# THU-luvision/TextureFusion

Measured on AMD Instinct MI355X. Metric: RGB-D frames/s (TSDF integrate + atlas update: prepare->integrate->finalize, UpdateMeshes, GeneratePatches + UpdateAtlas over the frame's dirty chunks), higher is better.
Workload: dtype f32

## Files before the change

texturefusion_amd/csrc/tf_devfn.h:

```cpp
#pragma once

#include "tf_device.h"

namespace tf {

__device__ __forceinline__ unsigned long long pack_id(int x, int y, int z) {
  return ((unsigned long long)((uint32_t)(x + (1 << 20)) & 0x1FFFFFu) << 42) |
         ((unsigned long long)((uint32_t)(y + (1 << 20)) & 0x1FFFFFu) << 21) |
         (unsigned long long)((uint32_t)(z + (1 << 20)) & 0x1FFFFFu);
}
__device__ __forceinline__ int4 unpack_id(unsigned long long k) {
  int4 r;
  r.x = (int)((k >> 42) & 0x1FFFFFu) - (1 << 20);
  r.y = (int)((k >> 21) & 0x1FFFFFu) - (1 << 20);
  r.z = (int)(k & 0x1FFFFFu) - (1 << 20);
  r.w = 0;
  return r;
}
__device__ __forceinline__ int part_key(const VolumeDev& v, int x, int y, int z) {
  return v.part_a * x + v.part_b * y + v.part_c * z;
}
__device__ __forceinline__ bool part_owned(const VolumeDev& v, int x, int y, int z) {
  const int k = part_key(v, x, y, z);
  return k >= v.part_lo && k < v.part_hi;
}
__device__ __forceinline__ bool part_band(const VolumeDev& v, int x, int y, int z) {
  const long long k = part_key(v, x, y, z);
  const long long s = v.part_a + v.part_b + v.part_c;
  return (k >= (long long)v.part_lo && k - (long long)v.part_lo <= s) || k == (long long)v.part_hi - 1;
}

__device__ __forceinline__ bool part_interior(const VolumeDev& v, int x, int y, int z) {
  const long long k = part_key(v, x, y, z);
  const long long s = (long long)v.part_a + v.part_b + v.part_c;
  return k - s >= (long long)v.part_lo && k + s < (long long)v.part_hi;
}

__device__ __forceinline__ uint32_t hash_key(unsigned long long k) {
  const unsigned long long h = k * 0x9E3779B97F4A7C15ull;
  return (uint32_t)(h >> 32) ^ (uint32_t)h;
}


__device__ __forceinline__ uint32_t hash_find(const VolumeDev& v, unsigned long long key) {
  uint32_t i = hash_key(key) & v.hmask;
  for (uint32_t probe = 0; probe <= v.hmask; ++probe) {
    const unsigned long long cur = v.hent[i].key;
    if (cur == key) return i;
    if (cur == kEmptyKey) return kInvalidSlot;
    i = (i + 1) & v.hmask;
  }
  return kInvalidSlot;
}

__device__ __forceinline__ uint32_t hash_slot_alive(const VolumeDev& v, unsigned long long key) {
  uint32_t i = hash_key(key) & v.hmask;
  for (uint32_t probe = 0; probe <= v.hmask; ++probe) {
    const uint4 e = *reinterpret_cast<const uint4*>(&v.hent[i]);
    const unsigned long long cur = ((unsigned long long)e.y << 32) | e.x;
    if (cur == key) return (e.w & 1u) ? e.z : kInvalidSlot;
    if (cur == kEmptyKey) return kInvalidSlot;
    i = (i + 1) & v.hmask;
  }
  return kInvalidSlot;
}

__device__ __forceinline__ uint32_t hash_slot_alive_ent(const VolumeDev& v, unsigned long long key, uint32_t* ent) {
  uint32_t i = hash_key(key) & v.hmask;
  for (uint32_t probe = 0; probe <= v.hmask; ++probe) {
    const uint4 e = *reinterpret_cast<const uint4*>(&v.hent[i]);
    const unsigned long long cur = ((unsigned long long)e.y << 32) | e.x;
    if (cur == key) { *ent = i; return (e.w & 1u) ? e.z : kInvalidSlot; }
    if (cur == kEmptyKey) return kInvalidSlot;
    i = (i + 1) & v.hmask;
  }
  return kInvalidSlot;
}

__device__ __forceinline__ uint32_t chunk_acquire(const VolumeDev& v, int4 id, bool* is_new,
                                               uint32_t* ent, const bool lazy = false) {
  const unsigned long long key = pack_id(id.x, id.y, id.z);
  uint32_t i = hash_key(key) & v.hmask;
  *is_new = true;
  for (uint32_t probe = 0; probe <= v.hmask; ++probe) {
    unsigned long long cur = v.hent[i].key;
    if (cur == kEmptyKey) {
      cur = atomicCAS(&v.hent[i].key, kEmptyKey, key);
      if (cur == kEmptyKey) {
        *ent = i;
        v.vctl->create_seq = v.seq;
        const uint32_t stripe = (hash_key(key) >> 7) & (kSlotStripes - 1);
        const uint32_t per = v.max_chunks / kSlotStripes;
        const uint32_t k = atomicAdd(&v.vctl->slot_cnt[stripe], 1u);
        const uint32_t slot = stripe * per + k;
        if (k >= per) {
          atomicOr(&v.vctl->status, kStPoolFull);
          v.hent[i].slot = kInvalidSlot;
          v.hent[i].alive = 0;
          return kInvalidSlot;
        }
        v.hent[i].slot = slot;
        v.hent[i].alive = 1;
        return slot;
      }
    }
    if (cur == key) {
      *ent = i;
      const uint32_t slot = v.hent[i].slot;
      if (slot == kInvalidSlot) return slot;
      if (!v.hent[i].alive) { if (!lazy) v.hent[i].alive = 1; }
      else *is_new = false;
      return slot;
    }
    i = (i + 1) & v.hmask;
  }
  atomicOr(&v.vctl->status, kStHashFull);
  *ent = 0;
  return kInvalidSlot;
}

__device__ __forceinline__ int nbr_word(int dx, int dy, int dz) { return (dx + 1) + 3 * (dy + 1) + 9 * (dz + 1); }
__device__ __forceinline__ uint32_t nbr_probe(const VolumeDev& v, unsigned long long key) {
  uint32_t i = hash_key(key) & v.hmask;
  for (uint32_t probe = 0; probe <= v.hmask; ++probe) {
    const uint4 e = *reinterpret_cast<const uint4*>(&v.hent[i]);
    const unsigned long long cur = ((unsigned long long)e.y << 32) | e.x;
    if (cur == key) return e.z + 1u;
    if (cur == kEmptyKey) return 0u;
    i = (i + 1) & v.hmask;
  }
  return 0u;
}
__device__ __forceinline__ uint32_t nbr_row_checked(const VolumeDev& v, const uint32_t own, const int4 id, const int lane,
                                                   uint32_t w, const uint32_t create_seq) {
  const uint32_t st = (uint32_t)__shfl((int)w, kNbrStamp);
  if (!(st > create_seq)) {
    if (lane < 27 && lane != 13 && w == 0u) {
      w = nbr_probe(v, pack_id(id.x + lane % 3 - 1, id.y + (lane / 3) % 3 - 1, id.z + lane / 9 - 1));
      if (w) v.nbr[(size_t)own * kNbrWords + lane] = w;
    }
    if (lane == kNbrStamp) v.nbr[(size_t)own * kNbrWords + lane] = v.seq;
  }
  return w;
}

constexpr uint32_t kBlkFail = 0x7FFFFFFFu;
__device__ __forceinline__ uint32_t blk_ring_mask(const VolumeDev& v, const int large) {
  uint32_t ns = v.mesh_blocks, nl = v.ovf_blocks;
  asm volatile("" : "+s"(ns), "+s"(nl));
  const uint32_t ms = ns > 2u ? (0xFFFFFFFFu >> __builtin_clz(ns - 1u)) : 1u;
  const uint32_t ml = nl > 2u ? (0xFFFFFFFFu >> __builtin_clz(nl - 1u)) : 1u;
  return large ? ml : ms;
}
__device__ __forceinline__ uint32_t* blk_ring(const VolumeDev& v, const int large) {
  uint32_t* const r = reinterpret_cast<uint32_t*>(v.mesh_rec + v.max_chunks);
// ... 88 lines not shown
```

texturefusion_amd/csrc/tf_kernels.hip:

```cpp
#include <stdlib.h>

#include <atomic>
#include "tf_device.h"
#include "tf_devfn.h"
#include "tf_devpose.h"
#include "tf_host_math.h"
#include "tf_patch_body.h"
#include "tf_voxel_math.h"

#pragma clang fp contract(off)
#ifndef TF_KA_GP
#define TF_KA_GP 2
#endif


namespace tf {

__global__ void k_reset_ctl(FrameCtl* ctl, VolCtl* vctl) {
  if (blockIdx.x == 0 && threadIdx.x == 0) {
    for (int a = 0; a < 3; ++a) {
      ctl->bbox_key[a] = f2key(1e8f);
      ctl->bbox_key[3 + a] = f2key(-1e8f);
      ctl->min_id[a] = ctl->max_id[a] = ctl->dims[a] = 0;
    }
// ... 432 lines not shown
    if (tile == n_tiles - 1u && threadIdx.x == 0) finish(tile_base + agg);
    __syncthreads();
  }
}
void launch_scan(const VolumeDev& v, int step, hipStream_t s) {
  static std::atomic<uint32_t> g_stamp{0};
  uint32_t stamp;
  do { stamp = (g_stamp.fetch_add(1u) + 1u) & 0x3FFFFFFFu; } while (stamp == 0u);
  hipLaunchKernelGGL(k_scan, dim3(256), dim3(256), 0, s, v, step, stamp);
}

__global__ __launch_bounds__(256) void k_acquire(VolumeDev v) {
  const SelBuf& L = v.sel;
  const uint32_t n = L.ctl->n_list;
  for (uint32_t e = blockIdx.x * 256 + threadIdx.x; e < n; e += gridDim.x * 256) {
    const int4 id = L.list_id[e];
    bool is_new = false;
    uint32_t ent = 0;
    const uint32_t slot = chunk_acquire(v, id, &is_new, &ent);
    L.list_slot[e] = slot;
    L.list_ent[e] = ent;
    L.list_new[e] = is_new ? 1 : 0;
    L.list_needs[e] = 0;
  }
}
void launch_acquire(const VolumeDev& v, hipStream_t s) {
  hipLaunchKernelGGL(k_acquire, dim3(512), dim3(256), 0, s, v);
}

__global__ __launch_bounds__(256) void k_pre(VolumeDev v, Pose P, Integ ig, float res, float resDiag, float4* out_pre,
                                             float* out_cen) {
  const SelBuf& L = v.sel;
  float4* pre = out_pre ? out_pre : L.list_pre;
  if (blockIdx.x == 0) centroid_table(P.p, res, out_cen ? out_cen : L.cen);
  const uint32_t n = L.ctl->n_list <= v.max_list ? L.ctl->n_list : 0u;
  for (uint32_t e = blockIdx.x * 256 + threadIdx.x; e < n; e += gridDim.x * 256) {
    const int4 id = L.list_id[e];
    const ChunkPre cp = chunk_pre(id, P.p, ig, res, resDiag);
    pre[4 * e] = make_float4(cp.a.x, cp.a.y, cp.a.z, cp.b.x);
    pre[4 * e + 1] = make_float4(cp.b.y, __int_as_float(id.x), __int_as_float(id.y), __int_as_float(id.z));
  }
}

__global__ __launch_bounds__(256) void k_lookup(VolumeDev v, uint32_t n) {
  const SelBuf& L = v.sel;
  const uint32_t i = blockIdx.x * 256 + threadIdx.x;
  if (i >= n) return;
  const int4 id = L.list_id[i];
  const uint32_t ent = hash_find(v, pack_id(id.x, id.y, id.z));
  uint32_t slot = kInvalidSlot;
  if (ent != kInvalidSlot && v.hent[ent].alive) slot = v.hent[ent].slot;
  if (slot == kInvalidSlot) atomicOr(&v.vctl->status, kStMissing);
  L.list_slot[i] = slot;
  L.list_ent[i] = (ent == kInvalidSlot) ? 0u : ent;
}
void launch_lookup(const VolumeDev& v, uint32_t n, hipStream_t s) {
  if (!n) return;
  hipLaunchKernelGGL(k_lookup, dim3((n + 255) / 256), dim3(256), 0, s, v, n);
}

#ifndef TF_KF_WAVES
#define TF_KF_WAVES 7
#endif
#ifndef TF_KFP_EXTRA
#define TF_KFP_EXTRA 1
#endif
#ifndef TF_KFP_WAVES
#define TF_KFP_WAVES 7
#endif

typedef uint32_t u32x4 __attribute__((ext_vector_type(4)));
typedef const __attribute__((address_space(4))) u32x4* const_u32x4_ptr;
typedef uint32_t u32x8 __attribute__((ext_vector_type(8)));
typedef const __attribute__((address_space(4))) u32x8* const_u32x8_ptr;

template <bool COLOR, bool QUALITY, bool FUSED, bool FLAG, int GP, bool TL = false>
__device__ __forceinline__ void integrate_body(const VolumeDev& v, const FrameImages& img, const Cam& cam,
                                               const IntegrateConsts& kc, const uint32_t epoch,
                                               const uint32_t bid, const uint32_t nb, const int claim_par = -1) {
  const SelBuf& L = v.sel;
  const int lane = threadIdx.x & 63;
  const uint32_t wave = (uint32_t)__builtin_amdgcn_readfirstlane((int)((bid * 256 + threadIdx.x) >> 6));
  const uint32_t nwaves = nb * 4;
  uint32_t n = L.ctl->n_list <= v.max_list ? L.ctl->n_list : 0u;
  uint32_t nf = n;
  if (FUSED) {
    const unsigned long long pk = L.ctl->emit_pack;
    nf = (uint32_t)pk;
    const unsigned long long tot = (pk & 0xFFFFFFFFull) + (pk >> 32);
    n = tot <= (unsigned long long)v.max_list ? (uint32_t)tot : 0u;
    if (!n) nf = 0;
    if (bid == 0 && threadIdx.x == 0) { L.ctl->n_list = n; L.ctl->n_front = nf; }
  }
  const uint32_t n_items = n;
  auto item_pos = [&](const uint32_t e) -> uint32_t { return FUSED ? list_phys(v, e, nf) : e; };
  const int vy = lane >> 3;
  const int W = cam.W, H = cam.H;
  if (FUSED && bid == 0 && threadIdx.x == 0) {
    for (int a = 0; a < 3; ++a) {
      L.ctl->bbox_key[a] = f2key(1e8f);
      L.ctl->bbox_key[3 + a] = f2key(-1e8f);
    }
  }

  const uint32_t e_first = wave, e_step = nwaves;
  u32x8 rec_next;
  {
    const uint32_t e0 = e_first < n_items ? e_first : 0u;
    const uint32_t p0 = n_items ? item_pos(e0) : 0u;
    rec_next = *(const_u32x8_ptr)(unsigned long long)(&L.list_pre[4 * (p0 < v.max_list ? p0 : 0u)]);
  }

  __shared__ float cenT[3][kChunkVoxels];
  {
    const float4* src = reinterpret_cast<const float4*>(L.cen);
    float4* dst = reinterpret_cast<float4*>(&cenT[0][0]);
    for (int i = threadIdx.x; i < 3 * kChunkVoxels / 4; i += 256) dst[i] = src[i];
  }
  __syncthreads();

  const __amdgpu_buffer_rsrc_t rs_depth =
      __builtin_amdgcn_make_buffer_rsrc((void*)img.depth, 0, W * H * 4, 0x00020000);
  const __amdgpu_buffer_rsrc_t rs_rgba =
      __builtin_amdgcn_make_buffer_rsrc((void*)img.rgba, 0, COLOR ? W * H * 4 : 0, 0x00020000);
  const __amdgpu_buffer_rsrc_t rs_qual =
      __builtin_amdgcn_make_buffer_rsrc((void*)img.quality, 0, QUALITY ? W * H * 4 : 0, 0x00020000);

  const uint32_t row_lo = lane < 32 ? (0xFFu << (lane & 24)) : 0u;
  const uint32_t row_hi = lane < 32 ? 0u : (0xFFu << (lane & 24));
  auto row_any = [&](const unsigned long long m) -> bool {
    return ((((uint32_t)m) & row_lo) | (((uint32_t)(m >> 32)) & row_hi)) != 0u;
  };
  auto ballot = [](const bool b) -> unsigned long long { return __builtin_amdgcn_ballot_w64(b); };

  float c_near = cam.nearP, c_far = cam.farP, c_thr = kc.thrCol, c_lower = kc.lower, c_sigma = kc.sigma;
  asm volatile("" : "+v"(c_near), "+v"(c_far), "+v"(c_thr), "+v"(c_lower), "+v"(c_sigma));

  if (TL && (kc.dbg & 8192u) && lane == 0 && wave < (uint32_t)kPhaseWaves)
  {
    v.phase_buf[wave * 16 + 14] = __builtin_amdgcn_s_memrealtime();
    v.phase_buf[wave * 16 + 8] = 0;
    v.phase_buf[wave * 16 + 9] = 0;
  }

  for (uint32_t e = e_first, e_next = e_first + e_step; e < n_items; e = e_next) {
    const uint32_t pe = item_pos(e);
    const u32x8 prw = rec_next;
    {
      e_next = e + e_step;
      const uint32_t en = e_next < n_items ? e_next : e;
      rec_next = *(const_u32x8_ptr)(unsigned long long)(&L.list_pre[4 * item_pos(en)]);
    }
    const int4 id = make_int4((int)prw[5], (int)prw[6], (int)prw[7], 0);
    const bool owned = part_owned(v, id.x, id.y, id.z);
    if (!owned) {
      if (FUSED && lane == 0) {
        L.list_slot[pe] = kInvalidSlot; L.list_ent[pe] = 0; L.list_new[pe] = 0; L.list_needs[pe] = 0;
        L.list_quality[pe] = 0.0f; L.list_rows[pe] = 0;
      }
      continue;
    }
    const unsigned long long key = pack_id(id.x, id.y, id.z);
    const uint32_t i0 = hash_key(key) & v.hmask;
    u32x4 h0 = {0u, 0u, 0u, 0u};
    uint32_t slot = kInvalidSlot;
    if (FUSED) h0 = *(const_u32x4_ptr)(unsigned long long)(&v.hent[i0]);
    else slot = L.list_slot[pe];
    bool is_new = false;
    uint32_t ent = i0;

    const float o0 = __uint_as_float(prw[0]), o1 = __uint_as_float(prw[1]), o2 = __uint_as_float(prw[2]);
    const float pbx = __uint_as_float(prw[3]), pby = __uint_as_float(prw[4]);
    const f32x2 o01 = {o0, o1};
    const f32x2 fxy = {cam.fxi, cam.fyi}, cxy = {kc.cxs, kc.cys};
    const float wD = FLAG ? pbx : -pbx;
    const float upper = pby;
    const float band = 32.0f * kc.res;
    const bool div_safe = (fabsf(o2) > band) && (fabsf(o2) < 1048576.0f) && (fabsf(o0) < 1048576.0f) &&
                          (fabsf(o1) < 1048576.0f) && (kc.res > 1e-6f) && (kc.res < 16.0f);
    if (TL && (kc.dbg & 8192u) && e == e_first && lane == 0 && wave < (uint32_t)kPhaseWaves) {
      asm volatile("" :: "s"(o0), "s"(o1), "s"(o2), "s"(id.x));
      v.phase_buf[wave * 16 + 15] = __builtin_amdgcn_s_memrealtime();
    }

    int off_d[8];
    int oobl[QUALITY ? 8 : 1];
    int oob_any = 0;
    uint32_t R = 64;
    unsigned long long all_valid = ~0ull;
    uint32_t oob_bits = 0;
    auto geometry = [&](auto safe_tag) {
      constexpr bool SAFE = decltype(safe_tag)::value;
#pragma unroll
      for (int j = 0; j < 8; ++j) {
        const int k = j * 64 + lane;
        const f32x2 pxy = o01 + (f32x2){cenT[0][k], cenT[1][k]};
        const float pzv = o2 + cenT[2][k];
        f32x2 q;
        if (SAFE) {
          q = div2_by(pxy, recip_refined(pzv));
// ... 799 lines not shown
```

texturefusion_amd/csrc/tf_mesh.hip:

```cpp
#include <stdlib.h>
#include <string.h>

#include <algorithm>
#include <vector>

#include "tf_devfn.h"
#include "tf_kf_store.h"
#include "tf_mc_table.h"
#include "tf_patch_body.h"
#include "tf_volume.h"

#pragma clang fp contract(off)

namespace tf {

__device__ const unsigned long long d_mc_tri[256] = TF_MC_TRI_TABLE_INIT;

constexpr int kR = 11;
constexpr int kRS = 11;
constexpr int kPS = kRS * kR;
constexpr int kRV = kPS * kR;
constexpr int kEdgeSlots = 3 * 729;
__device__ __forceinline__ uint32_t mesh_shard_rows_d(uint32_t max_chunks) { return max_chunks / kMeshShards + 258u; }

template <typename T>
__device__ __forceinline__ T load_here(const T* p) { return __hip_atomic_load(p, __ATOMIC_RELAXED, __HIP_MEMORY_SCOPE_WAVEFRONT); }

__device__ __forceinline__ int ridx(int x, int y, int z) { return (x + 1) + (y + 1) * kRS + (z + 1) * kPS; }

constexpr bool halo_needed(int rx, int ry, int rz) {
  if (rx < -1 || rx > 9 || ry < -1 || ry > 9 || rz < -1 || rz > 9) return false;
  if (rx >= 0 && rx < 8 && ry >= 0 && ry < 8 && rz >= 0 && rz < 8) return false;
  const int out = ((rx < 0 || rx > 8) ? 1 : 0) + ((ry < 0 || ry > 8) ? 1 : 0) + ((rz < 0 || rz > 8) ? 1 : 0);
  return out <= 1;
}
constexpr int count_halo_pairs() {
  int n = 0;
  for (int rz = -1; rz <= 9; ++rz)
    for (int ry = -1; ry <= 9; ++ry)
      for (int rx = -1; rx <= 9; ++rx) {
        if (!halo_needed(rx, ry, rz)) continue;
        const int vx = (rx + 8) & 7;
        if ((vx & 1) && halo_needed(rx - 1, ry, rz) && (((rx - 1 + 8) >> 3) == ((rx + 8) >> 3))) continue;
        ++n;
      }
  return n;
}
constexpr int kHalo = count_halo_pairs();
struct MeshTabs {
  unsigned long long halo[kHalo];
};
constexpr unsigned long long corner_of(int rx, int ry, int rz) {
  return (rx >= 0 && ry >= 0 && rz >= 0 && rx <= 8 && ry <= 8 && rz <= 8) ? (unsigned long long)(rx + ry * 9 + rz * 81 + 1) : 0ull;
}
constexpr MeshTabs make_mesh_tabs() {
  MeshTabs t{};
  int n = 0;
  for (int rz = -1; rz <= 9; ++rz)
    for (int ry = -1; ry <= 9; ++ry)
      for (int rx = -1; rx <= 9; ++rx) {
        if (!halo_needed(rx, ry, rz)) continue;
        const int vx = (rx + 8) & 7;
        const bool same_chunk_left = ((rx - 1 + 8) >> 3) == ((rx + 8) >> 3);
        if ((vx & 1) && halo_needed(rx - 1, ry, rz) && same_chunk_left) continue;
        const int rx0 = (vx & 1) ? rx - 1 : rx;
        const bool use0 = !(vx & 1);
        const bool use1 = (vx & 1) ? true : (halo_needed(rx + 1, ry, rz) && (((rx + 1 + 8) >> 3) == ((rx + 8) >> 3)));
        const int cx = (rx + 8) >> 3, cy = (ry + 8) >> 3, cz = (rz + 8) >> 3;
        const unsigned long long nb = (unsigned long long)(cx + cy * 3 + cz * 9);
        const unsigned long long pair = (unsigned long long)((((rx0 + 8) & 7) + ((ry + 8) & 7) * 8 + ((rz + 8) & 7) * 64) >> 1);
        const unsigned long long r0 = (unsigned long long)((rx0 + 1) + (ry + 1) * kRS + (rz + 1) * kPS);
        t.halo[n++] = (r0 & 2047ull) | (nb << 11) | (pair << 16) | ((use0 ? 1ull : 0ull) << 24) | ((use1 ? 1ull : 0ull) << 25) |
                      ((use0 ? corner_of(rx0, ry, rz) : 0ull) << 26) | ((use1 ? corner_of(rx0 + 1, ry, rz) : 0ull) << 36);
      }
  return t;
}
__device__ const MeshTabs d_mesh_tabs = make_mesh_tabs();

__device__ __forceinline__ int cox(int k) { return (0x66 >> k) & 1; }
__device__ __forceinline__ int coy(int k) { return (0xCC >> k) & 1; }
__device__ __forceinline__ int coz(int k) { return (0xF0 >> k) & 1; }
__device__ __forceinline__ int edge_c0(int e) { return (int)((0x321076543210ull >> (4 * e)) & 0xF); }
__device__ __forceinline__ int edge_c1(int e) { return (int)((0x765447650321ull >> (4 * e)) & 0xF); }

__device__ __forceinline__ int edge_slot(int x, int y, int z, int e) {
  const int bx = x + ((0x622 >> e) & 1);
  const int by = y + ((0xC44 >> e) & 1);
  const int bz = z + ((0x0F0 >> e) & 1);
  const int ax = e >= 8 ? 2 : (e & 1);
  return ax + (bx + by * 9 + bz * 81) * 3;
}
__device__ __forceinline__ int edge_of_slot(int ax, int dx, int dy, int dz) {
  if (ax == 0) return dz ? (dy ? 6 : 4) : (dy ? 2 : 0);
  if (ax == 1) return dz ? (dx ? 5 : 7) : (dx ? 1 : 3);
  return dy ? (dx ? 10 : 11) : (dx ? 9 : 8);
}

__device__ __forceinline__ bool gradient_at(const float* __restrict__ S, int px, int py, int pz, int ox, int oy,
                                            int oz, float res, float g[3]) {
  const int c = ridx(px, py, pz);
  const float xm = S[c - 1], xp = S[c + 1];
  const float ym = S[c - kRS], yp = S[c + kRS];
  const float zm = S[c - kPS], zp = S[c + kPS];
  const bool ok = ((ox ? xp : xm) < 1.0f) && ((oy ? yp : ym) < 1.0f) && ((oz ? zp : zm) < 1.0f);
  const float gx = xp - xm, gy = yp - ym, gz = zp - zm;
  const float yz = gy * gy + gz * gz;
  const float sq = gx * gx + yz;
  const float n = sqrtf(sq);
  g[0] = gx; g[1] = gy; g[2] = gz;
// ... 600 lines not shown
      unsigned long long usedm = 0;
      {
        constexpr int kWords = (kEpt * 4 + 31) / 32 + 1;
        const int w0 = first >> 3, sh0 = 4 * (first & 7);
#pragma unroll
        for (int q = 0; q < kWords; ++q) {
          const int wi = w0 + q;
          uint32_t x = wi < (kEdgeSlots + 7) / 8 ? sh.ownq[wi] : 0u;
          x |= x >> 1; x |= x >> 2; x &= 0x11111111u;
          x = (x | (x >> 3)) & 0x03030303u;
          x = (x | (x >> 6)) & 0x000F000Fu;
          x = (x | (x >> 12)) & 0xFFu;
          usedm |= (unsigned long long)x << (8 * q);
        }
        usedm >>= (sh0 >> 2);
        usedm &= (1ull << kEpt) - 1ull;
        const int left = kEdgeSlots - first;
        if (left < kEpt) usedm = left > 0 ? (usedm & ((1ull << left) - 1ull)) : 0ull;
      }
      const uint32_t cnt = (uint32_t)__popcll(usedm);
      uint32_t tc = 0;
#pragma unroll
      for (int j = 0; j < kCpt; ++j) tc += (uint32_t)sh.cinfo[kCpt * t + j] >> 12;
      uint32_t pk = cnt | (tc << 16);
      uint32_t inc = pk;
#pragma unroll
      for (int o = 1; o < 64; o <<= 1) {
        const uint32_t u = __shfl_up(inc, o);
        if (lane >= o) inc += u;
      }
      if (lane == 63) sh.wsum[w] = inc;
      __syncthreads();
      uint32_t before = 0, total = 0;
      for (int k = 0; k < NT / 64; ++k) {
        if (k < w) before += sh.wsum[k];
        total += sh.wsum[k];
      }
      if (t == 0) sh.ovf = mesh_block_for(v, sh.rblock, total & 0xFFFFu, total >> 16, sh.rpress);
      __syncthreads();
      const uint32_t ovf_blk = sh.ovf;
      uint16_t* const gvl = (ovf_blk != kBlkFail && (ovf_blk & kBlkLarge)) ? v.ovf_vlist + (size_t)((ovf_blk & ~kBlkLarge) - 1u) * kOvfCV : nullptr;
      const uint32_t excl = before + inc - pk;
      uint32_t r = excl & 0xFFFFu;
      sh.rbase[t] = (uint16_t)r;
      sh.rmask[t] = usedm;
      for (unsigned long long u = usedm; u; u &= u - 1ull) {
        const int m = first + (int)__builtin_ctzll(u);
        if (gvl) { if (r < (uint32_t)kOvfCV) gvl[r] = (uint16_t)m; }
        else if (r < v.mesh_cv) vlist[r] = (uint16_t)m;
        ++r;
      }
      uint32_t t0 = excl >> 16;
#pragma unroll
      for (int j = 0; j < kCpt; ++j) {
        sh.toff[kCpt * t + j] = (uint16_t)t0;
        t0 += (uint32_t)sh.cinfo[kCpt * t + j] >> 12;
      }
      if (t == 0) { sh.nv = total & 0xFFFFu; sh.nt = total >> 16; }
    }
    __syncthreads();
    const uint32_t nv = sh.nv, nt = sh.nt;
    const uint32_t ovf = sh.ovf;
    if (ovf == kBlkFail) {
      if (t == 0) {
        atomicOr(&v.vctl->status, kStMeshFull);
        const uint32_t was = sh.rstate & kMsInMap;
        rec->nv = 0; rec->nt = 0; rec->state = was | kMsOverflow; rec->epoch = epoch;
        if (rearm >= 0 && was) patch_list_append(v, rearm ^ 1, shard, id, own, sh.rtexloc, sh.rblock);
      }
      __syncthreads();
      continue;
    }
    const uint16_t* const gvlist = (ovf & kBlkLarge) ? v.ovf_vlist + (size_t)((ovf & ~kBlkLarge) - 1u) * kOvfCV : nullptr;

    if (DBG && dbg == 4) continue;
    if (DBG && dbg == 9) mesh_stamp(v, r, 6);
    const uint32_t inmap = (sh.rstate & kMsInMap) | (nv ? kMsInMap : 0u);
    if (t == NT - 64) {
      mesh_block_settle(v, sh.rblock, ovf);
      if (rearm >= 0 && inmap) patch_list_append(v, rearm ^ 1, shard, id, own, sh.rtexloc, ovf);
    }
    const float org[3] = {(float)(8 * id.x) * res, (float)(8 * id.y) * res, (float)(8 * id.z) * res};
    uint32_t adj = 0;
    for (uint32_t i = t; i < nv; i += NT) {
      const int m = gvlist ? gvlist[i] : vlist[i];
      const int cell = owner_cell(m, __builtin_ctz((sh.ownq[m >> 3] >> (4 * (m & 7))) & 0xFu));
      const int x = cell & 7, y = (cell >> 3) & 7, z = cell >> 6;
      const int ax = m % 3, b = m / 3;
      const int bx = b % 9, by = (b / 9) % 9, bz = b / 81;
      const int e = edge_of_slot(ax, bx - x, by - y, bz - z);
      const int e0 = edge_c0(e), e1 = edge_c1(e);
      const float s0 = sh.S[ridx(x + cox(e0), y + coy(e0), z + coz(e0))];
      const float s1 = sh.S[ridx(x + cox(e1), y + coy(e1), z + coz(e1))];
      const float tt = s0 / (s0 - s1);
      const int o0[3] = {cox(e0), coy(e0), coz(e0)}, o1[3] = {cox(e1), coy(e1), coz(e1)};
      const int cc[3] = {x, y, z};
      float pv[3];
#pragma unroll
      for (int a = 0; a < 3; ++a) {
        const float p0 = (float)o0[a] * res, p1 = (float)o1[a] * res;
        const float ev = p0 + tt * (p1 - p0);
        const float origin = org[a] + ((float)cc[a] * res + half);
        pv[a] = ev + origin;
      }
      const int k = (fabsf(s0) > fabsf(s1)) ? e1 : e0;
      const int px = x + cox(k), py = y + coy(k), pz = z + coz(k);
      float g[3];
      gradient_at(sh.S, px, py, pz, cox(k), coy(k), coz(k), res, g);
      const uint32_t cs = sh.nslot[((px + 8) >> 3) + ((py + 8) >> 3) * 3 + ((pz + 8) >> 3) * 9];
      const unsigned long long c4 = load_here(reinterpret_cast<const unsigned long long*>(v.color + (size_t)cs * kChunkVoxels + (px & 7) + (py & 7) * 8 + (pz & 7) * 64));
      float col[3] = {1.0f, 1.0f, 1.0f};
      const float cw = (float)(uint16_t)(c4 >> 48);
      if (cw > 0.0f) {
        col[0] = ((float)(uint16_t)c4 / 255.0f) / cw;
        col[1] = ((float)(uint16_t)(c4 >> 16) / 255.0f) / cw;
        col[2] = ((float)(uint16_t)(c4 >> 32) / 255.0f) / cw;
      }
#pragma unroll
      for (int a = 0; a < 3; ++a) {
        mesh_plane(v, ovf, kMpPos + a)[i] = pv[a];
        mesh_plane(v, ovf, kMpNrm + a)[i] = g[a];
        mesh_plane(v, ovf, kMpCol + a)[i] = col[a];
        const int gp = (int)floorf((pv[a] - org[a]) / (res * 1.0f));
        if (gp >= 8) adj |= 1u << (2 * a + 1);
        if (gp <= 0) adj |= 1u << (2 * a);
      }
    }
    if (adj) atomicOr(&sh.adj, adj);
    if (DBG && dbg == 9) mesh_stamp(v, r, 7);
    for (uint32_t ci = (uint32_t)(NT - 1 - t); ci < sh.ncell; ci += NT) {
      const int cell = sh.clist[ci];
      const uint32_t info = sh.cinfo[cell];
      if (!(info >> 12)) continue;
      const int x = cell & 7, y = (cell >> 3) & 7, z = cell >> 6;
      const unsigned long long row = d_mc_tri[sh.cidx[cell]];
      const uint32_t valid = info & 0xFFFu;
      uint32_t o = sh.toff[cell];
      for (int col = 0; col < 15; col += 3) {
        const int s0 = (int)((row >> (4 * col)) & 0xF);
        if (s0 == 0xF) break;
        const int s1 = (int)((row >> (4 * col + 4)) & 0xF), s2 = (int)((row >> (4 * col + 8)) & 0xF);
        if (!((valid >> s0) & (valid >> s1) & (valid >> s2) & 1u)) continue;
        constexpr int kEptT = 2304 / NT;
        auto ref_of = [&](int m) {
          const int tt = m / kEptT, j = m - tt * kEptT;
          return (uint16_t)(sh.rbase[tt] + (uint32_t)__popcll(sh.rmask[tt] & ((1ull << j) - 1ull)));
        };
        tri_plane(v, ovf, 0)[o] = ref_of(edge_slot(x, y, z, s2));
        tri_plane(v, ovf, 1)[o] = ref_of(edge_slot(x, y, z, s1));
        tri_plane(v, ovf, 2)[o] = ref_of(edge_slot(x, y, z, s0));
        ++o;
      }
    }
    __syncthreads();
    if (t == 0) {
      rec->nv = (uint16_t)nv; rec->nt = (uint16_t)nt; rec->epoch = epoch; rec->block = ovf;
      rec->state = inmap | (sh.adj << kMsAdjShift) | (inmap ? simplified : 0u);
    }
    __syncthreads();
    if (DBG && dbg == 9) mesh_stamp(v, r, 8);
  }
}

__global__ __launch_bounds__(256) void k_init_mesh_rec(MeshRec* rec, uint32_t n) {
  for (uint32_t i = blockIdx.x * 256 + threadIdx.x; i < n; i += gridDim.x * 256) {
    MeshRec r;
    memset(&r, 0, sizeof(r));
    r.texloc = kNoTexloc;
    r.frameid = -1;
    r.ratio[0] = r.ratio[1] = 1.0f;
    rec[i] = r;
  }
}
void launch_init_meshes(const VolumeDev& v, hipStream_t s) {
  hipLaunchKernelGGL(k_init_mesh_rec, dim3(1024), dim3(256), 0, s, v.mesh_rec, v.max_chunks);
  (void)hipMemsetAsync(v.mesh_rec + v.max_chunks, 0, sizeof(uint32_t) * ((size_t)blk_ring_len(v.mesh_blocks) + blk_ring_len(v.ovf_blocks)), s);
  (void)hipMemsetAsync(v.mesh_cnt, 0, sizeof(uint32_t) * 2 * kMeshCntWords, s);
}

uint32_t mesh_shard_rows(uint32_t max_chunks) { return max_chunks / kMeshShards + 258u; }

static void launch_mesher(const VolumeDev& v, int cnt_par, uint32_t max_entries, uint32_t epoch, float res, bool fused,
                          int rearm_set, hipStream_t s) {
  static const uint32_t dbg = getenv("TF_MESH_DBG") ? (uint32_t)atoi(getenv("TF_MESH_DBG")) : 0u;
  uint32_t* surv = v.mesh_nbr;
  uint32_t* cnt = v.mesh_cnt + (size_t)(cnt_par & 1) * kMeshCntWords;
  uint32_t* cnt_next = v.mesh_cnt + (size_t)((cnt_par & 1) ^ 1) * kMeshCntWords;
  const uint32_t cap_sh = mesh_shard_rows(v.max_chunks);
  uint32_t grid = ((max_entries + kMeshShards - 1) / kMeshShards + 1) * kMeshShards;
  static const uint32_t gmax = (uint32_t)device_cus() * (uint32_t)(TF_MESH_WAVES * 2);
  if (grid > gmax) grid = gmax;
  if (dbg)
    hipLaunchKernelGGL((k_mesh<128, true>), dim3(grid), dim3(128), v.mesh_cv * sizeof(uint16_t), s, v, surv, cnt, cnt_next, cap_sh, epoch, res,
// ... 522 lines not shown
```

texturefusion_amd/csrc/tf_patch_body.h:

```cpp
#pragma once

#include "tf_devfn.h"
#include "tf_device.h"

#pragma clang fp contract(off)

namespace tf {

__device__ __forceinline__ void rgb_at(const uint8_t* rgb, int stride, int W, int H, int y, int x, float c[3]) {
  const long i = (long)y * W + x;
  if (i < 0 || i >= (long)W * H) { c[0] = c[1] = c[2] = 0.0f; return; }
  const uint8_t* p = rgb + (size_t)i * stride;
  c[0] = (float)p[0]; c[1] = (float)p[1]; c[2] = (float)p[2];
}
__device__ __forceinline__ float f_at(const float* img, int W, int H, int y, int x) {
  const long i = (long)y * W + x;
  if (i < 0 || i >= (long)W * H) return 0.0f;
  return img[i];
}

__device__ __forceinline__ void bilinear_rgb(const uint8_t* rgb, int stride, int W, int H, float lx, float ly,
                                             float out[3]) {
  const int x = (int)floorf(lx), y = (int)floorf(ly);
  float c1[3], c2[3], c3[3];
// ... 135 lines not shown
    if (tl) {
      asm volatile("s_waitcnt vmcnt(0)" ::: "memory");
      if (lane == 0) v.phase_buf[wave * 16 + k] = __builtin_amdgcn_s_memrealtime();
    }
  };
  if (tl && lane == 0) v.phase_buf[wave * 16 + 0] = __builtin_amdgcn_s_memrealtime();
  const uint32_t shard = wave & (kMeshShards - 1u);
  const uint32_t shard_rows = mesh_shard_rows_dev(v.max_chunks);
  const int4* plist = v.patch_list + ((size_t)(par & 1) * kMeshShards + shard) * shard_rows;
  const uint32_t pe0 = FUSED ? wave / kMeshShards : wave;
  int4 e_first = make_int4(0, 0, 0, 0);
  if (FUSED) e_first = plist[pe0 < shard_rows ? pe0 : 0u];
  uint32_t n = S->n_work;
  if (FUSED) {
    n = v.patch_cnt[((par & 1) * kMeshShards + shard) * 16];
    if (n > shard_rows) n = shard_rows;
  }
  const uint32_t n_cand = FUSED ? S->n_cand : 0u;
  const unsigned long long slots_base = FUSED ? S->slots_base : 0ull;
  auto slots_room = [&](const unsigned long long base) -> unsigned long long {
    int aw = v.atlas_w, ah = v.atlas_h, pw = v.patch_w, ph = v.patch_h;
    asm volatile("" : "+s"(aw), "+s"(ah), "+s"(pw), "+s"(ph));
    const unsigned long long K = ((unsigned long long)aw + pw - 1) / (unsigned long long)pw;
    const unsigned long long bands = ((unsigned long long)ah + ph - 1) / (unsigned long long)ph;
    const unsigned long long total = K * bands;
    return total > base ? total - base : 0ull;
  };
  const unsigned long long room = FUSED ? slots_room(slots_base) : 0ull;
  const bool overflow = FUSED && (unsigned long long)n_cand > room;
  const int W = cam.W, H = cam.H;
  const float Wf = (float)W, Hf = (float)H;
  if (FUSED && bid == 0 && threadIdx.x == 0) {
    const unsigned long long got = (unsigned long long)n_cand < room ? (unsigned long long)n_cand : room;
    v.actl->n_slots = (uint32_t)(slots_base + got);
    if (overflow) atomicOr(&v.vctl->status, kStAtlasFull);
  }
  for (uint32_t pe = pe0; pe < n; pe += FUSED ? nwaves / kMeshShards : nwaves) {
    int4 id;
    uint32_t slot, lblk = kBlkNone;
    if (FUSED) {
      const int4 e = pe == pe0 ? e_first : plist[pe];
      id = unpack_id(((unsigned long long)(uint32_t)e.y << 32) | (uint32_t)e.x);
      slot = (uint32_t)e.z;
      lblk = (uint32_t)e.w;
    } else {
      id = v.work_ids[pe];
      slot = v.work_slot[pe];
    }
    if (slot == kInvalidSlot) continue;
    MeshRec* rec = &v.mesh_rec[slot];
    MeshRec R = *rec;
    const uint32_t mst = FUSED ? lblk : R.block;
    stampw(1);
    int xlane = lane;
    asm volatile("" : "+v"(xlane));
    const int xk = xlane < 6 ? xlane : 0, xm = xk ^ 1;
    uint32_t x_nw = 0u, x_bs = 0u;
    if (FUSED) {
      const int word = 13 + ((xk & 1) ? 1 : -1) * (xk < 2 ? 1 : (xk < 4 ? 3 : 9));
      x_nw = xlane < 6 ? v.nbr[(size_t)slot * kNbrWords + word] : 0u;
      x_bs = v.mesh_rec[x_nw ? x_nw - 1u : slot].state;
    }
    auto exchange_flags = [&]() {
      if (FUSED && x_nw != 0u && (x_bs & kMsInMap) && (x_bs & kMsSimplified)) {
        const uint32_t abit = 1u << (kMsAdjShift + xk), bbit = 1u << (kMsAdjShift + xm);
        const bool fa = (R.state & abit) != 0, fb = (x_bs & bbit) != 0;
        if (fa && !fb) atomicOr(&v.mesh_rec[x_nw - 1u].state, bbit);
        if (!fa && fb) atomicOr(&rec->state, abit);
      }
    };
    if (!PROJECT) exchange_flags();
    if (FUSED) {
      const bool cand = R.texloc == kNoTexloc;
      if (cand || overflow) {
        const unsigned long long key = pack_id(id.x, id.y, id.z);
        uint32_t c = 0;
        int l3 = lane;
        asm volatile("" : "+v"(l3));
        for (uint32_t i0 = 0; i0 < n_cand; i0 += 256) {
          unsigned long long ck[4];
#pragma unroll
          for (int q = 0; q < 4; ++q) {
            const uint32_t i = i0 + 64u * q + (uint32_t)l3;
            ck[q] = i < n_cand ? v.cand[i] : ~0ull;
          }
#pragma unroll
          for (int q = 0; q < 4; ++q) c += ck[q] < key ? 1u : 0u;
        }
#pragma unroll
        for (int o = 32; o >= 1; o >>= 1) c += (uint32_t)__shfl_xor((int)c, o);
        const AtlasCtl::Set* S2 = S;
        asm volatile("" : "+v"(S2));
        const unsigned long long base2 = S2->slots_base;
        if (overflow && (unsigned long long)c >= slots_room(base2) + (cand ? 0ull : 1ull)) { exchange_flags(); continue; }
        if (cand) {
          unsigned long long tl;
          if (!slot_texloc(v, base2 + c, &tl)) { exchange_flags(); continue; }
          R.texloc = tl;
          if (lane == 0) rec->texloc = tl;
        }
      }
    }
    stampw(2);
    const uint32_t nv = R.nv;
    const int kf_slot = FUSED ? -1 : (PROJECT ? id.w : R.kf_slot);
    if (!PROJECT && (!(R.pflags & kPfHasPatch) || kf_slot < 0)) continue;
    const KfDev kf = FUSED ? kf_fused : v.kf_tab[kf_slot];
    int bx = 0, by = 0, cols = 0, rows = 0;
    bool have_image = false;
    if (TL && FUSED && kf_fused.pad[0] == 2) { exchange_flags(); continue; }
    if (PROJECT) {
      float minX = Wf, maxX = 0.0f, minY = Hf, maxY = 0.0f;
      uint32_t dcmp = 0, ccmp = 0, ncau = 0;
      float* tu = mesh_plane(v, mst, kMpTc);
      float* tv = mesh_plane(v, mst, kMpTc + 1);
      float keepX[kVB], keepY[kVB];
      const bool one_sweep = nv <= 64u * kVB;
      for (uint32_t base = 0; base == 0 || base < nv; base += 64u * kVB) {
        float px[kVB], py[kVB], pz[kVB], m0[kVB], m1[kVB], m2[kVB];
        const uint32_t lim = base == 0 ? mesh_cap_v(v, mst) : nv;
        const uint32_t mld = mst != kBlkNone ? mst : 1u;
#pragma unroll
        for (int j = 0; j < kVB; ++j) {
          const uint32_t i = base + 64u * j + lane;
          const uint32_t ii = i < lim ? i : 0u;
          px[j] = mesh_plane(v, mld, kMpPos)[ii]; py[j] = mesh_plane(v, mld, kMpPos + 1)[ii];
          pz[j] = mesh_plane(v, mld, kMpPos + 2)[ii];
          m0[j] = mesh_plane(v, mld, kMpCol)[ii]; m1[j] = mesh_plane(v, mld, kMpCol + 1)[ii];
          m2[j] = mesh_plane(v, mld, kMpCol + 2)[ii];
        }
        if (base == 0) exchange_flags();
        stampw(3);
        float cX[kVB], cY[kVB], dist[kVB];
        Taps tp[kVB];
        uint32_t q1[kVB], q2[kVB], q3[kVB];
        float d1[kVB], d2[kVB], d3[kVB];
        bool cau[kVB];
#pragma unroll
        for (int j = 0; j < kVB; ++j) {
          float vl[3];
#pragma unroll
          for (int r = 0; r < 3; ++r) {
            float s = kf.T[4 * r] * px[j];
            s = s + kf.T[4 * r + 1] * py[j];
            s = s + kf.T[4 * r + 2] * pz[j];
            s = s + kf.T[4 * r + 3] * 1.0f;
            vl[r] = s;
          }
          dist[j] = vl[2];
          const float x = vl[0] / vl[2], y = vl[1] / vl[2];
          float a = (float)((double)(x * cam.fxi + cam.cxi) + 0.5);
          float b = (float)((double)(y * cam.fyi + cam.cyi) + 0.5);
          cau[j] = !(a >= 0 && a < Wf && b >= 0 && b < Hf);
          if (!(a >= 0)) a = 0;
          if (a >= Wf) a = Wf;
          if (!(b >= 0)) b = 0;
          if (b >= Hf) b = Hf;
          cX[j] = a; cY[j] = b;
          tp[j] = make_taps(W, H, a, b);
        }
#pragma unroll
        for (int j = 0; j < kVB; ++j) {
          q1[j] = load_px(kf.rgb, kf.stride, tp[j].i1);
          q2[j] = load_px(kf.rgb, kf.stride, tp[j].i2);
          q3[j] = load_px(kf.rgb, kf.stride, tp[j].i3);
          d1[j] = tp[j].i1 >= 0 ? kf.depth[tp[j].i1] : 0.0f;
          d2[j] = tp[j].i2 >= 0 ? kf.depth[tp[j].i2] : 0.0f;
          d3[j] = tp[j].i3 >= 0 ? kf.depth[tp[j].i3] : 0.0f;
        }
        stampw(4);
#pragma unroll
        for (int j = 0; j < kVB; ++j) {
          const uint32_t i = base + 64u * j + lane;
          const bool act = i < nv;
          bool cc = false, dc = false;
          if (act) {
// ... 49 lines not shown
        for (int j = 0; j < kVB; ++j) {
          const uint32_t i = 64u * j + lane;
          if (i < nv) { tu[i] = have_box ? keepX[j] - fbx : keepX[j]; tv[i] = have_box ? keepY[j] - fby : keepY[j]; }
        }
      } else if (have_box) {
        int l2 = lane;
        asm volatile("" : "+v"(l2));
        for (uint32_t i = (uint32_t)l2; i < nv; i += 64) {
          tu[i] = tu[i] - fbx;
          tv[i] = tv[i] - fby;
        }
      }
      if (lane == 0) {
        rec->bbox[0] = bx; rec->bbox[1] = by; rec->bbox[2] = cols; rec->bbox[3] = rows;
        rec->pflags = kPfHasPatch | kPfHasImage | (ncau ? kPfCaution : 0u) | (wrong ? kPfWrong : 0u);
        rec->ratio[0] = 1.0f; rec->ratio[1] = 1.0f;
        if (FUSED) { rec->frameid = kf.kf_id; rec->kf_slot = -1; }
      }
      have_image = true;
    } else {
      bx = R.bbox[0]; by = R.bbox[1]; cols = R.bbox[2]; rows = R.bbox[3];
      have_image = (R.pflags & kPfHasImage) != 0;
    }
    stampw(5);
    if (!BLIT) continue;
    if (TL && FUSED && kf_fused.pad[0] == 1) continue;
    if (!(nv > 0 && (R.state & kMsSimplified) && have_image && kf.kf_id >= 0)) continue;
    if (cols <= 0 || rows <= 0) continue;
    int PW = v.patch_w, PH = v.patch_h;
    asm volatile("" : "+s"(PW), "+s"(PH));
    float r0 = 1.0f, r1 = 1.0f;
    if (cols > PW) r0 = (float)PW / (float)cols;
    if (rows > PH) r1 = (float)PH / (float)rows;
    if (lane == 0) { rec->ratio[0] = r0; rec->ratio[1] = r1; }
    const unsigned long long tl = R.texloc;
    int aw_ = v.atlas_w;
    asm volatile("" : "+s"(aw_));
    const unsigned long long ox = tl % (unsigned long long)aw_, oy = tl / (unsigned long long)aw_;
    const size_t astep = (size_t)v.atlas_w * 3;
    const int st = kf.stride;
    if (r0 < 1 || r1 < 1) {
      if (ox + PW > (unsigned long long)v.atlas_w || oy + PH > (unsigned long long)v.atlas_h) continue;
      const double scale_x = 1.0 / ((double)PW / cols), scale_y = 1.0 / ((double)PH / rows);
      for (int t = lane; t < PW * PH; t += 64) {
        const int dy = t / PW, dx = t - dy * PW;
        float fx = (float)((dx + 0.5) * scale_x - 0.5);
        int sx = (int)floorf(fx);
        fx -= (float)sx;
        if (sx < 0) { fx = 0; sx = 0; }
        if (sx >= cols - 1) { fx = 0; sx = cols - 1; }
        const int a0 = (short)cv_round_f((1.f - fx) * 2048.f), a1 = (short)cv_round_f(fx * 2048.f);
        float fy = (float)((dy + 0.5) * scale_y - 0.5);
        int sy = (int)floorf(fy);
        fy -= (float)sy;
        int sy0 = sy, sy1 = sy + 1;
        sy0 = sy0 < 0 ? 0 : (sy0 > rows - 1 ? rows - 1 : sy0);
        sy1 = sy1 < 0 ? 0 : (sy1 > rows - 1 ? rows - 1 : sy1);
        const int b0 = (short)cv_round_f((1.f - fy) * 2048.f), b1 = (short)cv_round_f(fy * 2048.f);
        const int sx1 = sx + 1 < cols ? sx + 1 : sx;
        const uint32_t p00 = load_px(kf.rgb, st, (by + sy0) * W + bx + sx), p01 = load_px(kf.rgb, st, (by + sy0) * W + bx + sx1);
        const uint32_t p10 = load_px(kf.rgb, st, (by + sy1) * W + bx + sx), p11 = load_px(kf.rgb, st, (by + sy1) * W + bx + sx1);
        uint8_t* D = v.atlas + (oy + dy) * astep + (ox + dx) * 3;
#pragma unroll
        for (int k = 0; k < 3; ++k) {
          const int h0 = (int)((p00 >> (8 * k)) & 0xFFu) * a0 + (int)((p01 >> (8 * k)) & 0xFFu) * a1;
          const int h1 = (int)((p10 >> (8 * k)) & 0xFFu) * a0 + (int)((p11 >> (8 * k)) & 0xFFu) * a1;
          int val = (((b0 * (h0 >> 4)) >> 16) + ((b1 * (h1 >> 4)) >> 16) + 2) >> 2;
          val = val < 0 ? 0 : (val > 255 ? 255 : val);
          D[k] = (uint8_t)val;
        }
      }
    } else {
      if (ox + cols > (unsigned long long)v.atlas_w || oy + rows > (unsigned long long)v.atlas_h) continue;
      const int rowbytes = cols * 3;
      uint8_t* d0 = v.atlas + oy * astep + ox * 3;
      const int mis = (int)((uintptr_t)d0 & 3u);
      const bool rows_aligned = (astep & 3u) == 0;
      const int ndw = (rowbytes + mis + 3) >> 2;
      const float inv = 1.0f / (float)ndw;
      constexpr int kB = TF_PATCH_KB;
      for (int t0 = 0; t0 < rows * ndw; t0 += 64 * kB) {
        uint32_t val[kB];
        int off[kB], rr[kB];
#pragma unroll
        for (int k = 0; k < kB; ++k) {
          const int t = t0 + 64 * k + lane;
          const int r = (int)(((float)t + 0.5f) * inv);
          const int j = t - r * ndw;
          rr[k] = t < rows * ndw ? r : -1;
          const int o = 4 * j - (rows_aligned ? mis : (int)((uintptr_t)(d0 + (size_t)r * astep) & 3u));
          off[k] = o;
          uint32_t x = 0;
          if (rr[k] >= 0) {
            const uint8_t* srow = kf.rgb + ((size_t)(by + r) * W + bx) * st;
            if (st == 4) {
              const int p0 = (o > 0 ? o : 0) / 3;
              const uint32_t w0 = *reinterpret_cast<const uint32_t*>(srow + 4 * p0);
              const uint32_t w1 = (p0 + 1 < cols) ? *reinterpret_cast<const uint32_t*>(srow + 4 * (p0 + 1)) : 0u;
#pragma unroll
              for (int q = 0; q < 4; ++q) {
                const int bb = o + q;
                if (bb >= 0 && bb < rowbytes) {
                  const int px = bb / 3, ch = bb - 3 * px;
                  x |= (((px == p0 ? w0 : w1) >> (8 * ch)) & 0xFFu) << (8 * q);
                }
              }
            } else {
#pragma unroll
              for (int q = 0; q < 4; ++q) {
                const int bb = o + q;
                if (bb >= 0 && bb < rowbytes) {
                  const int px = bb / 3, ch = bb - 3 * px;
                  x |= (uint32_t)srow[px * st + ch] << (8 * q);
                }
              }
            }
          }
          val[k] = x;
        }
        stampw(6);
#pragma unroll
        for (int k = 0; k < kB; ++k) {
          if (rr[k] < 0) continue;
          uint8_t* drow = d0 + (size_t)rr[k] * astep;
          const int o = off[k];
          if (o >= 0 && o + 4 <= rowbytes) *reinterpret_cast<uint32_t*>(drow + o) = val[k];
          else {
#pragma unroll
            for (int q = 0; q < 4; ++q)
              if (o + q >= 0 && o + q < rowbytes) drow[o + q] = (uint8_t)(val[k] >> (8 * q));
          }
        }
      }
    }
  }
}

}
```

Before: 11170.

## Hoist and batch global loads across integrate, mesh and patch kernels to overlap latency

Several kernels have their global loads restructured so they are issued earlier and unconditionally, giving more memory-level parallelism. The integrate kernel loads the centroid table into registers before the list/bbox setup and only writes it to shared memory afterwards. The mesh kernel issues the color load before the interpolation math and reads packed 16-bit vertex lists as dwords. The patch kernel clamps candidate indices instead of branching, and its RGBA copy path issues all source-word loads for a batch before extracting bytes. Relaxed wavefront-scope atomic loads are used to keep the compiler from reordering or merging these loads. The cost is higher register pressure from holding more values live, plus a few redundant loads from clamped addresses.

```diff
diff --git a/texturefusion_amd/csrc/tf_devfn.h b/texturefusion_amd/csrc/tf_devfn.h
--- a/texturefusion_amd/csrc/tf_devfn.h
+++ b/texturefusion_amd/csrc/tf_devfn.h
@@ -36,6 +36,9 @@
   return k - s >= (long long)v.part_lo && k + s < (long long)v.part_hi;
 }
 
+template <typename T>
+__device__ __forceinline__ T load_here(const T* p) { return __hip_atomic_load(p, __ATOMIC_RELAXED, __HIP_MEMORY_SCOPE_WAVEFRONT); }
+
 __device__ __forceinline__ uint32_t hash_key(unsigned long long k) {
   const unsigned long long h = k * 0x9E3779B97F4A7C15ull;
   return (uint32_t)(h >> 32) ^ (uint32_t)h;
@@ -68,9 +71,9 @@
 __device__ __forceinline__ uint32_t hash_slot_alive_ent(const VolumeDev& v, unsigned long long key, uint32_t* ent) {
   uint32_t i = hash_key(key) & v.hmask;
   for (uint32_t probe = 0; probe <= v.hmask; ++probe) {
-    const uint4 e = *reinterpret_cast<const uint4*>(&v.hent[i]);
-    const unsigned long long cur = ((unsigned long long)e.y << 32) | e.x;
-    if (cur == key) { *ent = i; return (e.w & 1u) ? e.z : kInvalidSlot; }
+    const unsigned long long* const p = reinterpret_cast<const unsigned long long*>(&v.hent[i]);
+    const unsigned long long cur = load_here(p), sa = load_here(p + 1);
+    if (cur == key) { *ent = i; return ((uint32_t)(sa >> 32) & 1u) ? (uint32_t)sa : kInvalidSlot; }
     if (cur == kEmptyKey) return kInvalidSlot;
     i = (i + 1) & v.hmask;
   }
diff --git a/texturefusion_amd/csrc/tf_kernels.hip b/texturefusion_amd/csrc/tf_kernels.hip
--- a/texturefusion_amd/csrc/tf_kernels.hip
+++ b/texturefusion_amd/csrc/tf_kernels.hip
@@ -538,6 +538,13 @@
   const int lane = threadIdx.x & 63;
   const uint32_t wave = (uint32_t)__builtin_amdgcn_readfirstlane((int)((bid * 256 + threadIdx.x) >> 6));
   const uint32_t nwaves = nb * 4;
+  unsigned long long cen_ld[4];
+  {
+    const unsigned long long* const src = reinterpret_cast<const unsigned long long*>(L.cen);
+    const uint32_t t1 = threadIdx.x < 128u ? threadIdx.x + 256u : threadIdx.x;
+    cen_ld[0] = load_here(src + 2 * threadIdx.x); cen_ld[1] = load_here(src + 2 * threadIdx.x + 1);
+    cen_ld[2] = load_here(src + 2 * t1); cen_ld[3] = load_here(src + 2 * t1 + 1);
+  }
   uint32_t n = L.ctl->n_list <= v.max_list ? L.ctl->n_list : 0u;
   uint32_t nf = n;
   if (FUSED) {
@@ -569,9 +576,10 @@
 
   __shared__ float cenT[3][kChunkVoxels];
   {
-    const float4* src = reinterpret_cast<const float4*>(L.cen);
-    float4* dst = reinterpret_cast<float4*>(&cenT[0][0]);
-    for (int i = threadIdx.x; i < 3 * kChunkVoxels / 4; i += 256) dst[i] = src[i];
+    static_assert(3 * kChunkVoxels / 4 == 256 + 128, "the copy above: one float4 per thread and a second for the first 128");
+    unsigned long long* dst = reinterpret_cast<unsigned long long*>(&cenT[0][0]);
+    dst[2 * threadIdx.x] = cen_ld[0]; dst[2 * threadIdx.x + 1] = cen_ld[1];
+    if (threadIdx.x < 128u) { dst[2 * (threadIdx.x + 256u)] = cen_ld[2]; dst[2 * (threadIdx.x + 256u) + 1] = cen_ld[3]; }
   }
   __syncthreads();
 
diff --git a/texturefusion_amd/csrc/tf_mesh.hip b/texturefusion_amd/csrc/tf_mesh.hip
--- a/texturefusion_amd/csrc/tf_mesh.hip
+++ b/texturefusion_amd/csrc/tf_mesh.hip
@@ -23,8 +23,6 @@
 constexpr int kEdgeSlots = 3 * 729;
 __device__ __forceinline__ uint32_t mesh_shard_rows_d(uint32_t max_chunks) { return max_chunks / kMeshShards + 258u; }
 
-template <typename T>
-__device__ __forceinline__ T load_here(const T* p) { return __hip_atomic_load(p, __ATOMIC_RELAXED, __HIP_MEMORY_SCOPE_WAVEFRONT); }
 
 __device__ __forceinline__ int ridx(int x, int y, int z) { return (x + 1) + (y + 1) * kRS + (z + 1) * kPS; }
 
@@ -791,8 +789,16 @@
     }
     const float org[3] = {(float)(8 * id.x) * res, (float)(8 * id.y) * res, (float)(8 * id.z) * res};
     uint32_t adj = 0;
+    const bool vl_large = (__builtin_amdgcn_readfirstlane((int)ovf) & (int)kBlkLarge) != 0;
     for (uint32_t i = t; i < nv; i += NT) {
-      const int m = gvlist ? gvlist[i] : vlist[i];
+      int m;
+      if (vl_large) {
+        static_assert(kOvfCV % 2 == 0, "ovf_vlist is read as dwords");
+        m = (int)((load_here(reinterpret_cast<const uint32_t*>(gvlist) + (i >> 1)) >> (16u * (i & 1u))) & 0xFFFFu);
+        asm volatile("" : : "v"(m));
+      } else {
+        m = vlist[i];
+      }
       const int cell = owner_cell(m, __builtin_ctz((sh.ownq[m >> 3] >> (4 * (m & 7))) & 0xFu));
       const int x = cell & 7, y = (cell >> 3) & 7, z = cell >> 6;
       const int ax = m % 3, b = m / 3;
@@ -801,6 +807,10 @@
       const int e0 = edge_c0(e), e1 = edge_c1(e);
       const float s0 = sh.S[ridx(x + cox(e0), y + coy(e0), z + coz(e0))];
       const float s1 = sh.S[ridx(x + cox(e1), y + coy(e1), z + coz(e1))];
+      const int k = (fabsf(s0) > fabsf(s1)) ? e1 : e0;
+      const int px = x + cox(k), py = y + coy(k), pz = z + coz(k);
+      const uint32_t cs = sh.nslot[((px + 8) >> 3) + ((py + 8) >> 3) * 3 + ((pz + 8) >> 3) * 9];
+      const unsigned long long c4 = load_here(reinterpret_cast<const unsigned long long*>(v.color + (size_t)cs * kChunkVoxels + (px & 7) + (py & 7) * 8 + (pz & 7) * 64));
       const float tt = s0 / (s0 - s1);
       const int o0[3] = {cox(e0), coy(e0), coz(e0)}, o1[3] = {cox(e1), coy(e1), coz(e1)};
       const int cc[3] = {x, y, z};
@@ -812,12 +822,8 @@
         const float origin = org[a] + ((float)cc[a] * res + half);
         pv[a] = ev + origin;
       }
-      const int k = (fabsf(s0) > fabsf(s1)) ? e1 : e0;
-      const int px = x + cox(k), py = y + coy(k), pz = z + coz(k);
       float g[3];
       gradient_at(sh.S, px, py, pz, cox(k), coy(k), coz(k), res, g);
-      const uint32_t cs = sh.nslot[((px + 8) >> 3) + ((py + 8) >> 3) * 3 + ((pz + 8) >> 3) * 9];
-      const unsigned long long c4 = load_here(reinterpret_cast<const unsigned long long*>(v.color + (size_t)cs * kChunkVoxels + (px & 7) + (py & 7) * 8 + (pz & 7) * 64));
       float col[3] = {1.0f, 1.0f, 1.0f};
       const float cw = (float)(uint16_t)(c4 >> 48);
       if (cw > 0.0f) {
diff --git a/texturefusion_amd/csrc/tf_patch_body.h b/texturefusion_amd/csrc/tf_patch_body.h
--- a/texturefusion_amd/csrc/tf_patch_body.h
+++ b/texturefusion_amd/csrc/tf_patch_body.h
@@ -241,16 +241,16 @@
 #pragma unroll
           for (int q = 0; q < 4; ++q) {
             const uint32_t i = i0 + 64u * q + (uint32_t)l3;
-            ck[q] = i < n_cand ? v.cand[i] : ~0ull;
-          }
-#pragma unroll
-          for (int q = 0; q < 4; ++q) c += ck[q] < key ? 1u : 0u;
+            ck[q] = v.cand[i < n_cand ? i : 0u];
+          }
+#pragma unroll
+          for (int q = 0; q < 4; ++q) c += (i0 + 64u * q + (uint32_t)l3 < n_cand && ck[q] < key) ? 1u : 0u;
         }
 #pragma unroll
         for (int o = 32; o >= 1; o >>= 1) c += (uint32_t)__shfl_xor((int)c, o);
         const AtlasCtl::Set* S2 = S;
         asm volatile("" : "+v"(S2));
-        const unsigned long long base2 = S2->slots_base;
+        const unsigned long long base2 = ((const __attribute__((address_space(1))) AtlasCtl::Set*)S2)->slots_base;
         if (overflow && (unsigned long long)c >= slots_room(base2) + (cand ? 0ull : 1ull)) { exchange_flags(); continue; }
         if (cand) {
           unsigned long long tl;
@@ -466,30 +466,51 @@
       for (int t0 = 0; t0 < rows * ndw; t0 += 64 * kB) {
         uint32_t val[kB];
         int off[kB], rr[kB];
-#pragma unroll
-        for (int k = 0; k < kB; ++k) {
-          const int t = t0 + 64 * k + lane;
-          const int r = (int)(((float)t + 0.5f) * inv);
-          const int j = t - r * ndw;
-          rr[k] = t < rows * ndw ? r : -1;
-          const int o = 4 * j - (rows_aligned ? mis : (int)((uintptr_t)(d0 + (size_t)r * astep) & 3u));
-          off[k] = o;
-          uint32_t x = 0;
-          if (rr[k] >= 0) {
-            const uint8_t* srow = kf.rgb + ((size_t)(by + r) * W + bx) * st;
-            if (st == 4) {
-              const int p0 = (o > 0 ? o : 0) / 3;
-              const uint32_t w0 = *reinterpret_cast<const uint32_t*>(srow + 4 * p0);
-              const uint32_t w1 = (p0 + 1 < cols) ? *reinterpret_cast<const uint32_t*>(srow + 4 * (p0 + 1)) : 0u;
-#pragma unroll
-              for (int q = 0; q < 4; ++q) {
-                const int bb = o + q;
-                if (bb >= 0 && bb < rowbytes) {
-                  const int px = bb / 3, ch = bb - 3 * px;
-                  x |= (((px == p0 ? w0 : w1) >> (8 * ch)) & 0xFFu) << (8 * q);
-                }
+        if (st == 4) {
+          uint32_t w0[kB], w1[kB];
+#pragma unroll
+          for (int k = 0; k < kB; ++k) {
+            const int t = t0 + 64 * k + lane;
+            const int r = (int)(((float)t + 0.5f) * inv);
+            const int j = t - r * ndw;
+            const bool act = t < rows * ndw;
+            rr[k] = act ? r : -1;
+            const int o = 4 * j - (rows_aligned ? mis : (int)((uintptr_t)(d0 + (size_t)r * astep) & 3u));
+            off[k] = o;
+            const int p0 = act ? (o > 0 ? o : 0) / 3 : 0;
+            const int p1 = (act && p0 + 1 < cols) ? p0 + 1 : 0;
+            const uint8_t* srow = kf.rgb + ((size_t)(by + (act ? r : 0)) * W + bx) * 4;
+            w0[k] = load_here(reinterpret_cast<const uint32_t*>(srow + 4 * p0));
+            w1[k] = load_here(reinterpret_cast<const uint32_t*>(srow + 4 * p1));
+          }
+#pragma unroll
+          for (int k = 0; k < kB; ++k) {
+            const int o = off[k];
+            const int p0 = (o > 0 ? o : 0) / 3;
+            const uint32_t w1k = (p0 + 1 < cols) ? w1[k] : 0u;
+            uint32_t x = 0;
+#pragma unroll
+            for (int q = 0; q < 4; ++q) {
+              const int bb = o + q;
+              if (bb >= 0 && bb < rowbytes) {
+                const int px = bb / 3, ch = bb - 3 * px;
+                x |= (((px == p0 ? w0[k] : w1k) >> (8 * ch)) & 0xFFu) << (8 * q);
               }
-            } else {
+            }
+            val[k] = rr[k] >= 0 ? x : 0u;
+          }
+        } else {
+#pragma unroll
+          for (int k = 0; k < kB; ++k) {
+            const int t = t0 + 64 * k + lane;
+            const int r = (int)(((float)t + 0.5f) * inv);
+            const int j = t - r * ndw;
+            rr[k] = t < rows * ndw ? r : -1;
+            const int o = 4 * j - (rows_aligned ? mis : (int)((uintptr_t)(d0 + (size_t)r * astep) & 3u));
+            off[k] = o;
+            uint32_t x = 0;
+            if (rr[k] >= 0) {
+              const uint8_t* srow = kf.rgb + ((size_t)(by + r) * W + bx) * st;
 #pragma unroll
               for (int q = 0; q < 4; ++q) {
                 const int bb = o + q;
@@ -499,8 +520,10 @@
                 }
               }
             }
-          }
-          val[k] = x;
+            val[k] = x;
+          }
+#pragma unroll
+          for (int k = 0; k < kB; ++k) asm volatile("" : : "v"(val[k]));
         }
         stampw(6);
 #pragma unroll
```

Measured after the change: 10530. 5.7% lower.
